# PengfeiRen96/DIR

Measured on AMD Instinct MI355X. Metric: images/sec at 256x256 bs=64, 3 stage outputs (DIR.forward eval), higher is better.
Workload: dtype f16

## Files before the change

dir_amd/_capi.py:

```python
import ctypes as C
import os

_HERE = os.path.dirname(os.path.abspath(__file__))
LIB_PATH = os.environ.get('DIR_LIB_PATH') or os.path.join(_HERE, 'lib', 'libdir_hip.so')
_lib = None


class DirHipError(RuntimeError):
    pass


class ManoTables(C.Structure):
    _fields_ = [('shapedirs_t', C.c_void_p), ('posedirs_t', C.c_void_p), ('v_template', C.c_void_p),
                ('j_template', C.c_void_p), ('j_shapedirs', C.c_void_p), ('weights', C.c_void_p), ('hands_mean', C.c_void_p),
                ('comps', C.c_void_p), ('side', C.c_int32), ('center_idx', C.c_int32), ('root_palm', C.c_int32)]


class ManoFitHand(C.Structure):
    _fields_ = [(n, C.c_void_p) for n in ('p0', 'anchor', 'p_out', 'verts_t', 'joints_t', 'joints_conf', 'uv_t', 'uv_conf', 'verts', 'joints', 'joint_uv',
                                          'mse', 'status', 'state')]


class ManoFitOpts(C.Structure):
    _fields_ = [(n, C.c_float) for n in ('w_verts', 'w_joints', 'w_uv', 'w_pca', 'w_beta', 'w_init')] + [('lr', C.c_float * 4)] + [
# ... 24 lines not shown
class ConvSrc2(C.Structure):
    _fields_ = [(n, C.c_int32) for n in ('H', 'W', 'Cin', 'in_cstride', 'in_coff', 'stride')]


class TrainWeight(C.Structure):
    _fields_ = [(n, C.c_void_p) for n in ('w', 'fwd', 'fwd_scale', 'dgrad', 'dgrad_scale')] + [(n, C.c_int32) for n in ('Cout', 'Cin', 'kh', 'kw')] + [
        ('fwd_inv_in', C.c_float), ('dgrad_inv_in', C.c_float)]


class BneckChainParams(C.Structure):
    _fields_ = [(n, C.c_void_p) for n in ('w2', 'scale2', 'shift2', 'w3', 'scale3', 'shift3', 'w1n', 'scale1n', 'shift1n', 'wd')] + [
        ('n_next', C.c_int32), ('out_decimate', C.c_int32), ('dtype', C.c_int32)]


class BneckTailParams(C.Structure):
    _fields_ = [(n, C.c_void_p) for n in ('wstream', 'scale3', 'shift3', 'scale1n', 'shift1n')] + [('planes', C.c_int32), ('n_next', C.c_int32), ('waves', C.c_int32), ('dtype', C.c_int32)]


class ResChainParams(C.Structure):
    _fields_ = [(n, C.c_void_p) for n in ('w1', 'w2', 'w3', 'pre_scale', 'pre_shift', 'scale1', 'shift1', 'scale2', 'shift2', 'shift3')] + [
        (n, C.c_int32) for n in ('Cin', 'Cmid', 'Cout', 'dtype')]


class GemmDesc(C.Structure):
    _fields_ = [(n, C.c_int32) for n in ('M', 'N', 'K', 'lda', 'ldb', 'ldc', 'trans_a', 'trans_b', 'accumulate', 'batch')] + \
               [(n, C.c_int64) for n in ('stride_a', 'stride_b', 'stride_c')]


class GemmGroups(C.Structure):
    _fields_ = [(n, C.c_int32) for n in ('ny', 'nx', 'reduce', 'reserved')] + [(n, C.c_int64) for n in ('a_y', 'a_x', 'b_y', 'b_x', 'c_y', 'c_x')]


class TokenMlp(C.Structure):
    _fields_ = [(n, C.c_void_p) for n in ('w1t', 's1', 'b1', 'w2t', 'b2')]


class PgcnLayer(C.Structure):
    _fields_ = [(n, C.c_void_p) for n in ('W', 'e1', 'bias', 'bn_scale', 'bn_shift')] + [('relu', C.c_int32), ('w_dtype', C.c_int32)]


class SteBlock(C.Structure):
    _fields_ = [(n, C.c_void_p) for n in ('ln1_w', 'ln1_b', 'qkv_wt', 'qkv_b', 'proj_wt', 'proj_b', 'ln2_w', 'ln2_b',
                                          'fc1_wt', 'fc1_b', 'fc2_wt', 'fc2_b')]


class SteParams(C.Structure):
# ... 59 lines not shown
    _fields_ = [(n, C.c_void_p) for n in ('para', 'cam_px', 'raw_verts', 'raw_joints', 'raw_joints_px', 'smoothed', 'verts', 'joints', 'joints_px',
                                          'updated', 'state')]


class ManoParaSmoothOpts(C.Structure):
    _fields_ = [(n, C.c_double) for n in ('fps', 'min_cutoff', 'beta', 'd_cutoff', 'rot_speed_scale', 'cam_speed_scale')] + [
        ('max_gap', C.c_int32), ('shape_frames', C.c_int32)]


MANO_PARA_SMOOTH_FIELDS = ('measures', 'y1', 'y2', 'x1', 'x2', 'prev', 'vel', 'n_shape', 'age', 'run', 'count')


class GuardState(C.Structure):
    _fields_ = [('sumsq', C.c_double), ('norm', C.c_double), ('bc1', C.c_double), ('applied', C.c_longlong), ('skipped', C.c_longlong),
                ('skipped_in_row', C.c_longlong), ('clipped', C.c_longlong), ('coef', C.c_float), ('bc2_sqrt', C.c_float),
                ('nonfinite', C.c_int32), ('skip', C.c_int32), ('reserved', C.c_int32 * 2)]


class RenderLights(C.Structure):
    _fields_ = [('ambient', C.c_float * 3), ('diffuse', C.c_float * 3), ('specular', C.c_float * 3), ('location', C.c_float * 3),
                ('shininess', C.c_float)]


ABI_VERSION = 54
DT_F32, DT_BF16, DT_F16X3, DT_F16X1, DT_F16X3P, DT_F16X1P, DT_F16 = 0, 1, 3, 4, 5, 6, 7
CONV_RELU, CONV_PRE_RELU = 1, 2

_p, _i = C.c_void_p, C.c_int
_SIGNATURES = {
    'dir_abi_version': (C.c_int, []),
    'dir_last_error': (C.c_char_p, []),
    'dir_device_info': (C.c_int, [C.c_char_p, _i, C.POINTER(C.c_int)]),
    'dir_launch_log_reset': (None, []),
    'dir_launch_log_get': (C.c_int, [C.c_char_p, _i]),
    'dir_launch_log_note': (None, [C.c_char_p, C.c_longlong]),
    'dir_probe_launch': (C.c_longlong, [_i, _p, C.c_longlong, _i, _p]),
    'dir_conv2d_forward': (C.c_int, [C.POINTER(ConvDesc), _p, _p, _p, _p, _p, _p, _p, _p, _p]),
    'dir_conv2d_forward_stats': (C.c_int, [C.POINTER(ConvDesc), _p, _p, _p, _p, _p, _p, _p, _p, _p, C.POINTER(C.c_int), _p]),
    'dir_conv2d_forward_masked': (C.c_int, [C.POINTER(ConvDesc), _p, _p, _p, _p, _p, _p, _p, _p, _p, _p]),
    'dir_conv2d_forward_ex': (C.c_int, [C.POINTER(ConvDesc), _p, _p, _p, _p, _p, _p, _p, _p, _p, C.POINTER(ConvBnBwd), C.POINTER(C.c_int), _p]),
    'dir_add_upsampled': (C.c_int, [_p, _p, _i, _i, _i, _i, _i, _i, _i, _p]),
    'dir_fuse_sum': (C.c_int, [_p, _p, _p, _p, _i, _i, _i, _i, _i, _i, _i, _p]),
    'dir_pack_f16x3_weights': (C.c_int, [_p, _p, _p, _p, _i, _i, _p]),
    'dir_train_pack_conv_weights': (C.c_int, [_p, _p, _i, _i, _p]),
    'dir_gemm_f32_splitk_workspace_bytes': (C.c_longlong, [C.POINTER(GemmDesc)]),
    'dir_gemm_f32_splitk': (C.c_int, [C.POINTER(GemmDesc), _p, _p, _p, _p, _p, C.c_longlong, _p]),
    'dir_axpy_multi_f32': (C.c_int, [_p, _p, _p, _i, C.c_float, _p]),
    'dir_split_f16_forward': (C.c_int, [_p, _p, C.c_longlong, _i, _i, _i, _p, _p, _i, C.c_float, _i, _p]),
    'dir_stem_prep': (C.c_int, [_p, _p, _i, _i, _i, _i, _i, _i, _i, _p]),
    'dir_stem_prep_s2d': (C.c_int, [_p, _p, _i, _i, _i, _i, _i, _i, _p]),
    'dir_image_normalize_forward': (C.c_int, [_p, _p, C.POINTER(C.c_float), C.POINTER(C.c_float), _i, _i, _i, _p]),
    'dir_stem_prep_s2d_u8': (C.c_int, [_p, _p, C.POINTER(C.c_float), C.POINTER(C.c_float), _i, _i, _i, _i, _i, _i, _p]),
    'dir_adamw_step': (C.c_int, [_p, _p, _p, _p, C.c_longlong, C.c_double, C.c_double, C.c_double, C.c_double, C.c_double,
                                 C.c_longlong, _p]),
    'dir_grad_norm_workspace_bytes': (C.c_longlong, [C.c_longlong]),
    'dir_grad_guard': (C.c_int, [_p, C.c_longlong, C.c_double, _i, C.c_double, C.c_double, _p, C.c_longlong, _p, _p]),
    'dir_adamw_guarded_step': (C.c_int, [_p, _p, _p, _p, _p, C.c_longlong, C.c_double, C.c_double, C.c_double, C.c_double, C.c_double,
                                         C.c_double, _p, _p]),
    'dir_stage_losses_backward': (C.c_int, [C.POINTER(LossPred), C.POINTER(LossTarget), C.c_float, _p, C.POINTER(C.c_void_p * 2),
                                            C.POINTER(C.c_void_p * 2), C.POINTER(LossPredGrad), _i, _p]),
    'dir_dense_losses_backward_workspace_bytes': (C.c_longlong, [_i, _i]),
    'dir_dense_losses_backward': (C.c_int, [_p, _p, _p, _p, C.POINTER(C.c_float), C.c_float, _p, _p, C.c_longlong, _p, _p, _i, _i, _i, _i, _p]),
    'dir_stage_losses_forward': (C.c_int, [C.POINTER(LossPred), C.POINTER(LossTarget), C.c_float, _p, _p, _i, _p]),
    'dir_dense_losses_workspace_bytes': (C.c_longlong, [_i, _i]),
    'dir_dense_losses_forward': (C.c_int, [_p, _p, _p, _p, C.POINTER(C.c_float), C.c_float, _p, C.c_longlong, _p, _i, _i, _i, _i, _p]),
    'dir_bottleneck_chain_forward': (C.c_int, [C.POINTER(BneckChainParams), _p, _p, _p, _p, _p, _i, _i, _i, _p]),
    'dir_bottleneck_tail_forward': (C.c_int, [C.POINTER(BneckTailParams), _p, _p, _p, _p, C.c_longlong, _p]),
    'dir_residual_chain_supported': (C.c_int, [_i] * 11),
    'dir_residual_chain_forward': (C.c_int, [C.POINTER(ResChainParams), _p, _p, _i, _i, _i, _i, _i, _i, _i, _p]),
    'dir_stem_pool_forward': (C.c_int, [_p, _i, C.POINTER(C.c_float), C.POINTER(C.c_float), _p, _p, _p, _p, _i, _i, _i, _p]),
    'dir_stem_pool_forward_dt': (C.c_int, [_p, _i, _i, C.POINTER(C.c_float), C.POINTER(C.c_float), _p, _p, _p, _p, _i, _i, _i, _p]),
    'dir_maxpool3x3s2': (C.c_int, [_p, _p, _i, _i, _i, _i, _i, _p]),
    'dir_upsample2x_bilinear': (C.c_int, [_p, _p, _i, _i, _i, _i, _i, _i, _i, _p]),
    'dir_init_head_forward': (C.c_int, [C.POINTER(InitHeadParams), _p, _p, _p, _i, _p, _p, _p, _i, _i, _i, _i, _i, _p]),
    'dir_bone_proj_forward': (C.c_int, [_p, _p, _p, _p, _p, _p, _i, _i, C.c_float, _i, _p]),
    'dir_conv2d_dual_forward': (C.c_int, [C.POINTER(ConvDesc), _p, C.POINTER(ConvSrc2), _p, _p, _p, _p, _p]),
    'dir_conv2d_dual_scaled_forward': (C.c_int, [C.POINTER(ConvDesc), _p, C.POINTER(ConvSrc2), _p, _p, _p, _p, _p, _p]),
    'dir_conv1x1_stream_forward': (C.c_int, [C.POINTER(ConvDesc), _p, C.POINTER(ConvSrc2), _p, _p, _p, _p, _p, _p, _p, _p]),
    'dir_conv2d_as_supported': (C.c_int, [C.POINTER(ConvDesc), _i, _i]),
    'dir_conv2d_as_forward': (C.c_int, [C.POINTER(ConvDesc), _p, _p, _p, _p, _p, _p, _i, _i, _p]),
    'dir_conv2d_as_chain_supported': (C.c_int, [C.POINTER(ConvDesc), _i, _i]),
    'dir_conv2d_as_chain_forward': (C.c_int, [C.POINTER(ConvDesc), _p, _p, _p, _p, _p, _p, _p, _i, _i, _p, _i, _i, _i, _p]),
    'dir_conv2d_sparse_forward': (C.c_int, [C.POINTER(ConvDesc), _p, _p, _p, _p, _p, _p, _p, _p]),
    'dir_grid_tokens_forward': (C.c_int, [_p, _i, _i, _i, _i, _i, _p, _p, _p, _p, _p, C.POINTER(TokenMlp),
                                          C.POINTER(TokenMlp), C.POINTER(TokenMlp), _p, _p, _i, _p]),
    'dir_pgcn_stack_forward': (C.c_int, [C.POINTER(PgcnLayer), _i, _p, _p, _p, C.c_longlong, _p, _i, _p]),
    'dir_pgcn_stack_forward_pair': (C.c_int, [C.POINTER(PgcnLayer), C.POINTER(PgcnLayer), _i, _p, _p, _p, _p, _i, _p]),
    'dir_ste_forward': (C.c_int, [C.POINTER(SteParams), _p, _p, _p, _i, _p]),
    'dir_regress_forward': (C.c_int, [C.POINTER(RegressParams), _p, _p, _p, _p, _p, _p, _p, _p, _i, _p]),
    'dir_bone_fusion_scratch_bytes': (C.c_size_t, [_i]),
    'dir_bone_fusion_prepare': (C.c_int, [C.POINTER(BoneFusionParams), _p, _p, _i, _p]),
    'dir_bone_fusion_forward': (C.c_int, [C.POINTER(BoneFusionParams), _p, _p, _p, _p, _i, _i, C.c_float, _i, _i, _i, _p]),
# ... 71 lines not shown
    'dir_render_adjacency': (C.c_int, [_p, _p, C.c_longlong, _p]),
    'dir_render_vertex_normals': (C.c_int, [_p, _p, _p, _i, _p, _p]),
    'dir_render_shaded_workspace_bytes': (C.c_longlong, [_i]),
    'dir_render_joints': (C.c_int, [_p, _p, _p, _i, _i, C.c_float, C.c_float, _p]),
    'dir_render_shaded': (C.c_int, [_p, _p, _p, _p, _p, _p, _p, C.POINTER(RenderLights), _p, _i, _i, _p, C.c_longlong, _p, _p, _p, _p, _p, _p]),
    'dir_mesh_penetration': (C.c_int, [_p, _p, _p, _p, _i, _i, _i, _i, _i, _p, _p, _p, _p, _p, _p]),
    'dir_mesh_intersection_volume': (C.c_int, [_p, _p, _p, _p, _i, _i, _i, _i, _i, C.c_float, _i, _p, _p, _p, _p]),
    'dir_procrustes_align': (C.c_int, [_p, _p, _i, _i, _i, _p, _p, _p, _p]),
    'dir_point_set_nn': (C.c_int, [_p, _p, _i, _i, _i, _p, _p, _p]),
    'dir_threshold_counts': (C.c_int, [_p, C.c_longlong, _p, _i, _p, _p]),
    'dir_crop_matrices_from_boxes': (C.c_int, [_p, _i, C.c_double, _i, _p, _p, _p]),
    'dir_crop_matrices_from_meshes': (C.c_int, [_p, _p, _p, _p, _p, _i, C.c_double, _i, _p, _p, _p]),
    'dir_crop_frames': (C.c_int, [_p, C.c_longlong, _p, _p, _p, _i, _i, _p, _p, _p]),
    'dir_crop_frames_area': (C.c_int, [_p, C.c_longlong, _p, _p, _p, _i, _i, _p, _p, _p, _p]),
    'dir_one_euro_state_bytes': (C.c_longlong, [_i, _i, C.POINTER(C.c_longlong)]),
    'dir_one_euro_step': (C.c_int, [_p, _p, _i, C.POINTER(OneEuroSegment), _i, C.c_double, C.c_double, C.c_double, C.c_double, _i, _p, _p, _p, _p]),
    'dir_mano_para_smooth_state_bytes': (C.c_longlong, [C.POINTER(C.c_longlong)]),
    'dir_mano_para_smooth_step': (C.c_int, [C.POINTER(ManoTables), C.POINTER(ManoParaSmoothHand), _p, C.POINTER(ManoParaSmoothOpts), _i, _i, _p]),
}


PROFILE = None
_pending = {}
_NO_PROFILE = ('dir_conv2d_as_supported', 'dir_conv2d_as_chain_supported', 'dir_residual_chain_supported', 'dir_abi_version', 'dir_last_error', 'dir_device_info', 'dir_launch_log_reset', 'dir_launch_log_get', 'dir_launch_log_note',
               'dir_bone_fusion_scratch_bytes', 'dir_dense_losses_workspace_bytes', 'dir_dense_losses_backward_workspace_bytes',
               'dir_gemm_f32_splitk_workspace_bytes', 'dir_bn_train_workspace_bytes', 'dir_bn_sync_workspace_bytes', 'dir_bn_frozen_workspace_bytes', 'dir_jpeg_planes_bytes', 'dir_render_workspace_bytes', 'dir_render_adjacency_bytes', 'dir_render_shaded_workspace_bytes', 'dir_colsum_workspace_bytes', 'dir_conv2d_wgrad_workspace_bytes', 'dir_conv2d_wgrad_f16x3_workspace_bytes',
               'dir_one_euro_state_bytes', 'dir_mano_para_smooth_state_bytes', 'dir_grad_norm_workspace_bytes')


def annotate(**kw):
    if PROFILE is not None:
        _pending.update(kw)


class _ProfLib(object):
    def __init__(self, l):
        self._l = l

    def __getattr__(self, name):
        fn = getattr(self._l, name)
        if name in _NO_PROFILE:
            return fn
        import torch

        def call(*args):
            e0, e1 = torch.cuda.Event(enable_timing=True), torch.cuda.Event(enable_timing=True)
            self._l.dir_launch_log_reset()
# ... 58 lines not shown
```

dir_amd/engine.py:

```python
import ctypes as C
import math
import json
import os
import threading

import torch

from . import _capi
from ._capi import CONV_PRE_RELU, CONV_RELU, DT_BF16, DT_F16, DT_F16X1, DT_F16X1P, DT_F16X3, DT_F16X3P, DT_F32, ConvDesc
from .packing import pack_as_weights, pack_stream_weights, pack_tail_stream

F32 = torch.float32
IMAGENET_MEAN = (C.c_float * 3)(0.485, 0.456, 0.406)
IMAGENET_STD = (C.c_float * 3)(0.229, 0.224, 0.225)
class _ThreadState(threading.local):
    variant = None
    arith = None
    capture = None
    capture_fused = None
    calibrating = False
    no_out_split = False


_TLS = _ThreadState()


def _variant_for(op, B):
    return _TLS.variant if _TLS.variant is not None else op.variant.get(B, 0)


def _packing_arith():
    return _TLS.arith

# ... 359 lines not shown
    @staticmethod
    def applies(c3, c1n, dtype):
        return (dtype in HALF and c3.kh == 1 and c3.stride == 1 and c3.scale is not None and c3.cout == 4 * c3.cin
                and c1n.kh == 1 and c1n.stride == 1 and c1n.cin == c3.cout and c1n.scale is not None and c1n.pre_scale is None
                and (c3.cin, c1n.cout) in BneckTailOp.GEOMETRIES)

    def __call__(self, y2, x):
        B, H, W, P = y2.shape
        M = B * H * W
        if _TLS.capture_fused is not None:
            _TLS.capture_fused.append((self, (y2, x), {}))
        out = torch.empty(B, H, W, self.c3.cout, device=y2.device, dtype=y2.dtype)
        y1n = torch.empty(B, H, W, self.c1n.cout, device=y2.device, dtype=y2.dtype)
        if _capi.PROFILE is not None:
            c4, n2 = self.c3.cout, self.c1n.cout
            _capi.annotate(family='conv', flops=2.0 * M * (P * c4 + c4 * n2), op=self, dtype='bf16',
                           shape='M=%d tail 1x1(%d->%d)+res+1x1(->%d)' % (M, P, c4, n2),
                           bytes=(M * (P + 2 * c4 + n2) + c4 * P + n2 * c4) * 2)
        _capi.check(_capi.lib().dir_bottleneck_tail_forward(C.byref(self.params), _capi.ptr(y2), _capi.ptr(x), _capi.ptr(out), _capi.ptr(y1n), M,
                                                            _capi.stream_ptr()), 'dir_bottleneck_tail_forward')
        return out, y1n


def stem_conv_op(w, scale, shift, dtype):
    wp = torch.zeros(64, 64, 4, 1, device=w.device, dtype=F32)
    for r in range(4):
        for dy in range(2):
            ky = 2 * r + dy - 1
            if not 0 <= ky <= 6:
                continue
            for j in range(4):
                for dx in range(2):
                    kx = 2 * j + dx - 1
                    if 0 <= kx <= 6:
                        c0 = j * 16 + (dy * 2 + dx) * 4
                        wp[:, c0:c0 + 3, r, 0] = w[:, :, ky, kx]
    op = ConvOp(wp, dtype, stride=1, pad=0, scale=scale, shift=shift, relu=True)
    op.ho = op.wo = 128
    op.in_cs_override = 16
    op.alg_k = 147
    return op


class BackboneOp(object):
    fused_stem = os.environ.get('DIR_FUSED_STEM', '1') != '0'
    bneck_chain = os.environ.get('DIR_BNECK_CHAIN', '1') != '0'
    bneck_tail = os.environ.get('DIR_BNECK_TAIL', '1') != '0'

    def __init__(self, sd, p, dtype, device):
        dt = self.dtype = dtype
        self.device = device
        w = sd[p + '.conv1.weight']
        wk = torch.zeros(64, 7, 8, 4, device=w.device, dtype=F32)
        wk[:, :, :7, :3] = w.permute(0, 2, 3, 1)
        self.stem_w = wk.to(dtype if dtype in HALF else torch.bfloat16).contiguous().to(device)
        s_, h_ = bn_fold(sd, p + '.bn1')
        self.stem_scale, self.stem_shift = s_.float().contiguous().to(device), h_.float().contiguous().to(device)
        self.stem = stem_conv_op(sd[p + '.conv1.weight'], s_, h_, dt)
        self.layers = []
        for li, n in enumerate((3, 4, 6, 3), start=1):
            blocks = []
            for b in range(n):
                q = '%s.layer%d.%d' % (p, li, b)
                stride = 2 if (b == 0 and li > 1) else 1
                s1, h1 = bn_fold(sd, q + '.bn1')
                s2, h2 = bn_fold(sd, q + '.bn2')
                s3, h3 = bn_fold(sd, q + '.bn3')
                blk = dict(c1=ConvOp(sd[q + '.conv1.weight'], dt, scale=s1, shift=h1, relu=True),
                           c2=ConvOp(sd[q + '.conv2.weight'], dt, stride=stride, pad=1, scale=s2, shift=h2, relu=True),
                           c3=ConvOp(sd[q + '.conv3.weight'], dt, scale=s3, shift=h3, relu=True))
# ... 5 lines not shown
                    blk['c2'].link_split(blk['c3'])
                blocks.append(blk)
            self.layers.append(blocks)
        if self.bneck_chain:
            l1 = self.layers[0]
            for i, blk in enumerate(l1):
                nxt = l1[i + 1]['c1'] if i + 1 < len(l1) else self.layers[1][0]['c1']
                if 'dual' in blk:
                    if BneckChainOp.applies(blk['c2'], None, nxt, dt, dual=blk['dual']):
                        blk['chain'] = BneckChainOp(blk['c2'], None, nxt, dual=blk['dual'])
                elif BneckChainOp.applies(blk['c2'], blk['c3'], nxt, dt):
                    blk['chain'] = BneckChainOp(blk['c2'], blk['c3'], nxt)

        if self.bneck_tail:
            for li in (1, 2):
                blocks = self.layers[li]
                for i, blk in enumerate(blocks):
                    if 'dual' in blk or 'chain' in blk:
                        continue
                    nxt = blocks[i + 1]['c1'] if i + 1 < len(blocks) else self.layers[li + 1][0]['c1']
                    if BneckTailOp.applies(blk['c3'], nxt, dt):
                        blk['tail'] = BneckTailOp(blk['c3'], nxt)

    def __call__(self, img):
        L, dt, dev = _capi.lib(), self.dtype, self.device
        B = img.shape[0]
        if self.fused_stem and dt in HALF:
            x = torch.empty(B, 64, 64, 64, device=dev, dtype=dt)
            u8 = img.dtype == torch.uint8
            _ann('stem', 2.0 * B * 128 * 128 * 64 * 147, img.numel() * img.element_size() + x.numel() * 2 + self.stem_w.numel() * 2,
                 'B=%d 7x7/2 conv + bn + relu + maxpool' % B)
            _capi.check(L.dir_stem_pool_forward_dt(_capi.ptr(img), 2 if u8 else 0, _dt(dt), IMAGENET_MEAN, IMAGENET_STD, _capi.ptr(self.stem_w),
                                                _capi.ptr(self.stem_scale), _capi.ptr(self.stem_shift), _capi.ptr(x), B, 256, 256,
                                                _capi.stream_ptr()), 'dir_stem_pool_forward')
            return self._layers(x)
        Hs, Ws = 131, 132
        xp = torch.empty(B, Hs, Ws, 16, device=dev, dtype=dt)
        _ann('stem', 0, img.numel() * img.element_size() + xp.numel() * xp.element_size(), 'B=%d space-to-depth staging' % B)
        if img.dtype == torch.uint8:
            _capi.check(L.dir_stem_prep_s2d_u8(_capi.ptr(img), _capi.ptr(xp), IMAGENET_MEAN, IMAGENET_STD, B, 256, 256, Hs, Ws,
                                               _dt(dt), _capi.stream_ptr()), 'dir_stem_prep_s2d_u8')
        else:
            _capi.check(L.dir_stem_prep_s2d(_capi.ptr(img), _capi.ptr(xp), B, 256, 256, Hs, Ws, _dt(dt), _capi.stream_ptr()),
                        'dir_stem_prep_s2d')
        s1 = self.stem(xp)
        x = torch.empty(B, 64, 64, 64, device=dev, dtype=dt)
        _ann('stem', 0, (s1.numel() + x.numel()) * x.element_size(), 'B=%d maxpool 3x3/2' % B)
        _capi.check(L.dir_maxpool3x3s2(_capi.ptr(s1), _capi.ptr(x), B, 128, 128, 64, _dt(dt), _capi.stream_ptr()),
                    'dir_maxpool3x3s2')
        return self._layers(x)

    decimate_c1 = os.environ.get('DIR_DECIMATE_C1', '1') != '0'

    def _layers(self, x):
        feats = []
        y1 = None
        x_dec = False
        for li, blocks in enumerate(self.layers):
            for bi, blk in enumerate(blocks):
                if 'chain' in blk:
                    dec = (self.decimate_c1 and li == 0 and bi == len(blocks) - 1 and blk['chain'].c1n is not None and 'dual' in self.layers[1][0]
                           and self.layers[1][0]['dual'].stride2 == 2 and 'chain' not in self.layers[1][0] and not _TLS.no_out_split)
                    x, y1 = blk['chain'](y1 if y1 is not None else blk['c1'](x), x, decimate=dec)
                    x_dec = dec
                    continue
                if 'tail' in blk and (x.shape[0] * x.shape[1] * x.shape[2]) % 64 == 0:
                    x, y1 = blk['tail'](blk['c2'](y1 if y1 is not None else blk['c1'](x)), x)
                elif 'dual' in blk:
                    x, y1 = blk['dual'](blk['c2'](y1 if y1 is not None else blk['c1'](x)), x, x_decimated=x_dec), None
                    x_dec = False
                else:
                    x, y1 = blk['c3'](blk['c2'](y1 if y1 is not None else blk['c1'](x)), residual=x), None
            feats.append(None if x_dec else x)
        return feats


def backbone_standalone(module, x, compute_dtype=torch.float32):
    _capi.require_cuda(x)
    if module.training:
        raise NotImplementedError('dir_amd implements the inference path (eval-mode BatchNorm); call .eval()')
    sd = {'b.' + k: v.detach() for k, v in module.state_dict().items()}
    op = BackboneOp(sd, 'b', compute_dtype, x.device)
    op.decimate_c1 = False
    with torch.cuda.device(x.device):
        feats = op(_capi.f32c(x.detach()))
    return [f.permute(0, 3, 1, 2).float() for f in feats]


# ... 810 lines not shown
```

dir_amd/packing.py:

```python
import torch


def pack_as_weights(w_ohwi, A):
    N, kh, kw, Cin = w_ohwi.shape
    assert N % (128 * A) == 0 and Cin % 64 == 0
    nt = kh * kw
    dev = w_ohwi.device
    w = w_ohwi.reshape(N, nt * Cin)
    lane = torch.arange(64, device=dev)
    l32, h = lane & 31, lane >> 5
    e = torch.arange(8, device=dev)
    g, wv, st, ks, cb = torch.meshgrid(torch.arange(N // (128 * A), device=dev), torch.arange(4, device=dev), torch.arange(nt * Cin // 64, device=dev),
                                       torch.arange(4, device=dev), torch.arange(A, device=dev), indexing='ij')
    row = (g * (128 * A) + (wv * A + cb) * 32)[..., None] + l32
    slab, tap = st // nt, st % nt
    k0 = (tap * Cin + 64 * slab + 8 * ks)[..., None] + 32 * h
    return w[row[..., None], k0[..., None] + e].contiguous()


def pack_stream_weights(w_nk, dtype=torch.bfloat16):
    N, K = w_nk.shape
    assert N % 128 == 0 and K % 64 == 0
    return pack_as_weights(w_nk.detach().to(dtype).reshape(N, 1, 1, K), 2 if N % 256 == 0 else 1)


def pack_tail_stream(w3, w1n, waves=8, dtype=torch.bfloat16):
    out_dev = w3.device
    w3 = w3.detach().float().reshape(w3.shape[0], -1).cpu()
    w1n = w1n.detach().float().reshape(w1n.shape[0], -1).cpu()
    C4, P = w3.shape
    N2 = w1n.shape[0]
    assert w1n.shape[1] == C4 and C4 == 4 * P and C4 % 512 == 0 and N2 in (128, 256)
    dev = w3.device
    lane = torch.arange(64, device=dev)
    l32, h, l16, g16 = lane & 31, lane >> 5, lane & 15, lane >> 4
    e = torch.arange(8, device=dev)
    KBS = P // 16
    out = []
    if waves == 4:
        ncc = N2 // 128
        for hf in range(C4 // 512):
            for w in range(4):
                for cb in range(4):
                    for ks in range(KBS):
                        out.append(w3[(hf * 512 + 128 * w + 32 * cb + l32)[:, None], (16 * ks + 8 * h)[:, None] + e])
                for ks in range(32):
# ... 18 lines not shown
```

include/dir_hip.h:

```cpp
#ifndef DIR_HIP_H
#define DIR_HIP_H

#include <stddef.h>
#include <stdint.h>

#ifdef __cplusplus
extern "C" {
#endif

#define DIR_OK 0
#define DIR_E_INVALID (-1)
#define DIR_E_LAUNCH (-2)
#define DIR_E_NODEVICE (-3)

#define DIR_ABI_VERSION 54

int dir_abi_version(void);
const char* dir_last_error(void);
int dir_device_info(char* arch_host, int arch_len, int* num_cu_host);
void dir_launch_log_reset(void);
int dir_launch_log_get(char* buf_host, int len);
void dir_launch_log_note(const char* name, long long times);
long long dir_probe_launch(int mode, void* buf, long long bytes, int iters, void* stream);

typedef struct dir_mano_tables {
    const float* shapedirs_t;
    const float* posedirs_t;
    const float* v_template;
    const float* j_template;
    const float* j_shapedirs;
    const float* weights;
    const float* hands_mean;
    const float* comps;
    int32_t side;
    int32_t center_idx;
    int32_t root_palm;
} dir_mano_tables;

// ... 392 lines not shown
    const float* scale1n; const float* shift1n;
    int32_t planes;
    int32_t n_next;
    int32_t waves;
    int32_t dtype;
} dir_bneck_tail_params;
int dir_bottleneck_tail_forward(const dir_bneck_tail_params* p, const void* y2, const void* residual, void* out, void* y1_next,
                                long long M, void* stream);

typedef struct dir_res_chain_params {
    const void* w1; const void* w2; const void* w3;
    const float* pre_scale; const float* pre_shift;
    const float* scale1; const float* shift1;
    const float* scale2; const float* shift2;
    const float* shift3;
    int32_t Cin, Cmid, Cout;
    int32_t dtype;
} dir_res_chain_params;
int dir_residual_chain_supported(int dtype, int Cin, int Cmid, int Cout, int B, int H, int W, int in_cstride, int in_coff, int out_cstride,
                                 int out_coff);
int dir_residual_chain_forward(const dir_res_chain_params* p, const void* x, void* out, int B, int H, int W, int in_cstride, int in_coff,
                               int out_cstride, int out_coff, void* stream);

typedef struct dir_loss_pred {
    const float* joint_uv[2];
    const float* mesh_uv[2];
    const float* proj[2];
    const float* joint_xyz[2];
    const float* mesh_xyz[2];
    const float* offset;
} dir_loss_pred;
typedef struct dir_loss_target {
    const float* joint_2d[2];
    const float* mesh_2d[2];
    const float* joint_3d[2];
    const float* mesh_3d[2];
    const float* center[2];
    const int32_t* faces[2];
    int32_t c2, n_faces;
} dir_loss_target;
int dir_stage_losses_forward(const dir_loss_pred* pred_host, const dir_loss_target* gt_host, float coord_weight, double* scratch,
                             float* out13, int B, void* stream);
long long dir_dense_losses_workspace_bytes(int B, int S);
int dir_dense_losses_forward(const float* seg_logits, const float* dense_pred, const float* gt_seg, const float* gt_dense,
                             const float* class_weight_host, float dense_weight, void* workspace, long long workspace_bytes,
                             float* out3, int B, int S, int H, int W, void* stream);
// ... 166 lines not shown
```

Before: 28200.

## Fuse layer3 bottleneck 3x3 conv, 1x1 expand, residual and next 1x1 into one kernel

Adds a persistent HIP kernel for layer3 bottleneck blocks (256 planes, 16-wide maps). It computes the 3x3 conv on a haloed row patch in LDS, then the 1x1 expand with BN, residual add and ReLU, then optionally the next block's 1x1 reduce, all in one kernel. Weights are streamed through a register ring and tiles are kept in LDS. This removes the intermediate y2 global round-trip and several launches per block. In exchange the kernel is highly specialized, with large LDS use and one block per CU, and falls back to the old path when the shape is unsupported.

```diff
diff --git a/dir_amd/_capi.py b/dir_amd/_capi.py
--- a/dir_amd/_capi.py
+++ b/dir_amd/_capi.py
@@ -70,6 +70,11 @@
         (n, C.c_int32) for n in ('Cin', 'Cmid', 'Cout', 'dtype')]
 
 
+class BneckBlockParams(C.Structure):
+    _fields_ = [(n, C.c_void_p) for n in ('wstream', 'scale2', 'shift2', 'scale3', 'shift3', 'scale1n', 'shift1n')] + [
+        (n, C.c_int32) for n in ('planes', 'n_next', 'dtype')]
+
+
 class GemmDesc(C.Structure):
     _fields_ = [(n, C.c_int32) for n in ('M', 'N', 'K', 'lda', 'ldb', 'ldc', 'trans_a', 'trans_b', 'accumulate', 'batch')] + \
                [(n, C.c_int64) for n in ('stride_a', 'stride_b', 'stride_c')]
@@ -175,7 +180,7 @@
                 ('shininess', C.c_float)]
 
 
-ABI_VERSION = 54
+ABI_VERSION = 55
 DT_F32, DT_BF16, DT_F16X3, DT_F16X1, DT_F16X3P, DT_F16X1P, DT_F16 = 0, 1, 3, 4, 5, 6, 7
 CONV_RELU, CONV_PRE_RELU = 1, 2
 
@@ -221,6 +226,8 @@
     'dir_bottleneck_tail_forward': (C.c_int, [C.POINTER(BneckTailParams), _p, _p, _p, _p, C.c_longlong, _p]),
     'dir_residual_chain_supported': (C.c_int, [_i] * 11),
     'dir_residual_chain_forward': (C.c_int, [C.POINTER(ResChainParams), _p, _p, _i, _i, _i, _i, _i, _i, _i, _p]),
+    'dir_bottleneck_block_supported': (C.c_int, [_i] * 6),
+    'dir_bottleneck_block_forward': (C.c_int, [C.POINTER(BneckBlockParams), _p, _p, _p, _p, _i, _i, _i, _p]),
     'dir_stem_pool_forward': (C.c_int, [_p, _i, C.POINTER(C.c_float), C.POINTER(C.c_float), _p, _p, _p, _p, _i, _i, _i, _p]),
     'dir_stem_pool_forward_dt': (C.c_int, [_p, _i, _i, C.POINTER(C.c_float), C.POINTER(C.c_float), _p, _p, _p, _p, _i, _i, _i, _p]),
     'dir_maxpool3x3s2': (C.c_int, [_p, _p, _i, _i, _i, _i, _i, _p]),
@@ -338,7 +345,7 @@
 
 PROFILE = None
 _pending = {}
-_NO_PROFILE = ('dir_conv2d_as_supported', 'dir_conv2d_as_chain_supported', 'dir_residual_chain_supported', 'dir_abi_version', 'dir_last_error', 'dir_device_info', 'dir_launch_log_reset', 'dir_launch_log_get', 'dir_launch_log_note',
+_NO_PROFILE = ('dir_conv2d_as_supported', 'dir_conv2d_as_chain_supported', 'dir_residual_chain_supported', 'dir_bottleneck_block_supported', 'dir_abi_version', 'dir_last_error', 'dir_device_info', 'dir_launch_log_reset', 'dir_launch_log_get', 'dir_launch_log_note',
                'dir_bone_fusion_scratch_bytes', 'dir_dense_losses_workspace_bytes', 'dir_dense_losses_backward_workspace_bytes',
                'dir_gemm_f32_splitk_workspace_bytes', 'dir_bn_train_workspace_bytes', 'dir_bn_sync_workspace_bytes', 'dir_bn_frozen_workspace_bytes', 'dir_jpeg_planes_bytes', 'dir_render_workspace_bytes', 'dir_render_adjacency_bytes', 'dir_render_shaded_workspace_bytes', 'dir_colsum_workspace_bytes', 'dir_conv2d_wgrad_workspace_bytes', 'dir_conv2d_wgrad_f16x3_workspace_bytes',
                'dir_one_euro_state_bytes', 'dir_mano_para_smooth_state_bytes', 'dir_grad_norm_workspace_bytes')
diff --git a/dir_amd/csrc/l3_chain.hip b/dir_amd/csrc/l3_chain.hip
--- /dev/null
+++ b/dir_amd/csrc/l3_chain.hip
@@ -0,0 +1,323 @@
+#include "conv_common.h"
+
+namespace dir {
+namespace {
+
+using convk::bf16_t;
+using convk::f16s_t;
+using convk::f32x16;
+using convk::Half;
+
+constexpr int P = 256, C4 = 1024;
+constexpr int TM = 64;
+constexpr int HC = 512;
+constexpr int NTHR = 512;
+constexpr int TPITCH = HC * 2 + 16;
+constexpr int YPITCH = P * 2 + 16;
+constexpr int PROW = 9728;
+constexpr int PATCH = 6 * PROW;
+constexpr int R0 = TM * TPITCH > PATCH ? TM * TPITCH : PATCH;
+constexpr int GRP = 8;
+constexpr int NAF = 144;
+constexpr int NBF = 32;
+
+struct L3Args {
+    const bf16_t* y1; const bf16_t* res; bf16_t* out; bf16_t* y1n;
+    const uint4* wstream;
+    const float* sc2; const float* sh2; const float* sc3; const float* sh3; const float* sc1n; const float* sh1n;
+    int H, tiles_per_img, ntiles;
+};
+
+template <typename H> __device__ __forceinline__ void unpack4(uint2 v, float (&f)[4]) {
+    convk::unpack2<H>(v.x, f[0], f[1]);
+    convk::unpack2<H>(v.y, f[2], f[3]);
+}
+
+template <int V> struct IC : std::integral_constant<int, V> {};
+
+template <int N2, typename H>
+__global__ __launch_bounds__(NTHR, 1) void l3_chain_kernel(L3Args a) {
+    convk::half_kernel_init<H>();
+    constexpr bool NEXT = N2 != 0;
+    constexpr int NCF = NEXT ? HC / 16 : 0;
+    constexpr int NUF = NBF + NCF;
+    constexpr int NF = NAF + 2 * NUF;
+    constexpr int NGA = NAF / GRP, NGU = NUF / GRP;
+    static_assert(NAF % (2 * GRP) == 0 && NUF % (2 * GRP) == 0 && (N2 == 0 || N2 == 256), "l3_chain_kernel: the ring slot of a group must be compile-time");
+    __shared__ __attribute__((aligned(16))) char s_r0[R0];
+    __shared__ __attribute__((aligned(16))) char s_y2[TM * YPITCH];
+    __shared__ __attribute__((aligned(16))) float s_ss[2 * P + 2 * C4 + 2 * N2 + 4];
+    char* const s_t = s_r0;
+    const int tid = threadIdx.x, lane = tid & 63, wave = __builtin_amdgcn_readfirstlane(tid >> 6);
+    const int l32 = lane & 31, h = lane >> 5;
+
+    const int nblk = gridDim.x;
+    int t0, tstep, tend;
+    if ((nblk & 7) == 0 && a.ntiles % 8 == 0) {
+        const int per = a.ntiles >> 3;
+        t0 = (blockIdx.x & 7) * per + (blockIdx.x >> 3); tstep = nblk >> 3; tend = ((blockIdx.x & 7) + 1) * per;
+    } else { t0 = blockIdx.x; tstep = nblk; tend = a.ntiles; }
+    if (t0 >= tend) return;
+
+    const __amdgpu_buffer_rsrc_t wrs = __builtin_amdgcn_make_buffer_rsrc((void*)a.wstream, 0, 8 * NF * 1024, 0x00020000);
+    const int wv = (wave * NF * 64 + lane) * 16;
+    convk::u32x4 ring[2][GRP];
+    auto ring_load = [&](auto Slot, auto F0) {
+        constexpr int slot = decltype(Slot)::value, f0 = decltype(F0)::value;
+#pragma unroll
+        for (int i = 0; i < GRP; ++i) ring[slot][i] = __builtin_bit_cast(convk::u32x4, __builtin_amdgcn_raw_buffer_load_b128(wrs, wv, (f0 + i) * 1024, 0));
+    };
+    ring_load(IC<0>{}, IC<0>{});
+
+    for (int i = tid; i < P; i += NTHR) { s_ss[i] = a.sc2[i]; s_ss[P + i] = a.sh2[i]; }
+    for (int i = tid; i < C4; i += NTHR) { s_ss[2 * P + i] = a.sc3[i]; s_ss[2 * P + C4 + i] = a.sh3[i]; }
+    if constexpr (NEXT) {
+        for (int i = tid; i < N2; i += NTHR) { s_ss[2 * P + 2 * C4 + i] = a.sc1n[i]; s_ss[2 * P + 2 * C4 + N2 + i] = a.sh1n[i]; }
+    }
+    const float* const s_sc3 = s_ss + 2 * P;
+    const float* const s_sh3 = s_ss + 2 * P + C4;
+
+    uint4 xr[2][2][2];
+    auto res_fetch = [&](int tile, int half) {
+#pragma unroll
+        for (int pb = 0; pb < 2; ++pb) {
+            const bf16_t* rp = a.res + ((long long)tile * TM + 32 * pb + l32) * C4 + half * HC + 64 * wave + 8 * h;
+#pragma unroll
+            for (int cb = 0; cb < 2; ++cb)
+#pragma unroll
+                for (int j = 0; j < 2; ++j) xr[cb][pb][j] = *reinterpret_cast<const uint4*>(rp + 32 * cb + 16 * j);
+        }
+    };
+
+    f32x16 accc[2];
+    uint4 bop[2][2];
+    auto act_read = [&](auto F, auto Set) {
+        constexpr int f = decltype(F)::value, set = decltype(Set)::value;
+        if constexpr (f < NBF) {
+            constexpr int ks = f % 16;
+            constexpr int koff = NEXT ? 32 * ks : 128 * (ks >> 2) + 16 * (ks & 3);
+#pragma unroll
+            for (int pb = 0; pb < 2; ++pb)
+                bop[set][pb] = *reinterpret_cast<const uint4*>(s_y2 + (32 * pb + l32) * YPITCH + koff + (NEXT ? 16 : 64) * h);
+        } else {
+            constexpr int fc = f - NBF;
+#pragma unroll
+            for (int pb = 0; pb < 2; ++pb) bop[set][pb] = *reinterpret_cast<const uint4*>(s_t + (32 * pb + l32) * TPITCH + 32 * fc + 16 * h);
+        }
+    };
+
+    for (int t = t0; t < tend; t += tstep) {
+        const int img = t / a.tiles_per_img, trow = (t - img * a.tiles_per_img) * 4;
+
+        {
+            const int px = tid >> 5, ch = tid & 31;
+            uint4 pv[6];
+#pragma unroll
+            for (int i = 0; i < 6; ++i) {
+                const int iy = trow - 1 + i, iyc = min(max(iy, 0), a.H - 1);
+                pv[i] = *reinterpret_cast<const uint4*>(a.y1 + (((long long)img * a.H + iyc) * 16 + px) * P + ch * 8);
+                if (iy != iyc) pv[i] = make_uint4(0u, 0u, 0u, 0u);
+            }
+            res_fetch(t, 0);
+#pragma unroll
+            for (int i = 0; i < 6; ++i) *reinterpret_cast<uint4*>(s_r0 + i * PROW + (px + 1) * YPITCH + ch * 16) = pv[i];
+            if (tid < 384) *reinterpret_cast<uint4*>(s_r0 + (tid >> 6) * PROW + ((tid >> 5) & 1) * 17 * YPITCH + ch * 16) = make_uint4(0u, 0u, 0u, 0u);
+        }
+        __syncthreads();
+
+        {
+            f32x16 acc[2];
+#pragma unroll
+            for (int j = 0; j < 2; ++j)
+#pragma unroll
+                for (int r = 0; r < 16; ++r) acc[j][r] = 0.f;
+            const char* bB = s_r0 + (l32 >> 4) * PROW + (l32 & 15) * YPITCH + 64 * h;
+            auto bread = [&](auto I) {
+                constexpr int i = decltype(I)::value, s = i >> 2, ks = i & 3, slab = s / 9, tap = s % 9, ky = tap / 3, kx = tap % 3;
+#pragma unroll
+                for (int j = 0; j < 2; ++j) bop[i & 1][j] = *reinterpret_cast<const uint4*>(bB + (ky + 2 * j) * PROW + kx * YPITCH + slab * 128 + 16 * ks);
+            };
+            bread(IC<0>{});
+            [&]<int... G>(std::integer_sequence<int, G...>) {
+                (([&] {
+                     constexpr int grp = G, slot = G & 1;
+                     __builtin_amdgcn_sched_barrier(0);
+                     ring_load(IC<slot ^ 1>{}, IC<(G + 1) * GRP>{});
+                     [&]<int... I>(std::integer_sequence<int, I...>) {
+                         (([&] {
+                              constexpr int i = grp * GRP + I;
+                              if constexpr (i + 1 < NAF) bread(IC<i + 1>{});
+                              __builtin_amdgcn_sched_barrier(0);
+#pragma unroll
+                              for (int j = 0; j < 2; ++j) acc[j] = Half<H>::mfma32(ring[slot][I], bop[i & 1][j], acc[j]);
+                          }()),
+                          ...);
+                     }(std::make_integer_sequence<int, GRP>{});
+                 }()),
+                 ...);
+            }(std::make_integer_sequence<int, NGA>{});
+#pragma unroll
+            for (int j = 0; j < 2; ++j)
+#pragma unroll
+                for (int q = 0; q < 4; ++q) {
+                    const int c0 = 32 * wave + 8 * q + 4 * h;
+                    const float4 sc = *reinterpret_cast<const float4*>(s_ss + c0);
+                    const float4 sh = *reinterpret_cast<const float4*>(s_ss + P + c0);
+                    uint2 o;
+                    o.x = Half<H>::pack2_relu(fmaf(acc[j][4 * q], sc.x, sh.x), fmaf(acc[j][4 * q + 1], sc.y, sh.y));
+                    o.y = Half<H>::pack2_relu(fmaf(acc[j][4 * q + 2], sc.z, sh.z), fmaf(acc[j][4 * q + 3], sc.w, sh.w));
+                    *reinterpret_cast<uint2*>(s_y2 + (32 * j + l32) * YPITCH + c0 * 2) = o;
+                }
+        }
+        __syncthreads();
+
+        auto unit = [&](auto HF) {
+            constexpr int hf = decltype(HF)::value;
+            constexpr bool last_half = hf == 1;
+            constexpr int fbase = NAF + hf * NUF;
+            f32x16 accb[2];
+            if constexpr (NEXT && hf == 0) {
+#pragma unroll
+                for (int pb = 0; pb < 2; ++pb)
+#pragma unroll
+                    for (int r = 0; r < 16; ++r) accc[pb][r] = 0.f;
+            }
+            act_read(IC<0>{}, IC<0>{});
+            [&]<int... G>(std::integer_sequence<int, G...>) {
+                (([&] {
+                     constexpr int grp = G, slot = G & 1;
+                     constexpr int fnext = G + 1 < NGU ? fbase + (G + 1) * GRP : last_half ? 0 : fbase + NUF;
+                     ring_load(IC<slot ^ 1>{}, IC<fnext>{});
+                     [&]<int... I>(std::integer_sequence<int, I...>) {
+                         (([&] {
+                              constexpr int f = grp * GRP + I, set = f & 1;
+                              if constexpr (f + 1 < NUF && f + 1 != NBF) act_read(IC<f + 1>{}, IC<set ^ 1>{});
+                              if constexpr (f < NBF) {
+                                  constexpr int cb = f / 16, ks = f - cb * 16;
+                                  if constexpr (ks == 0) {
+#pragma unroll
+                                      for (int pb = 0; pb < 2; ++pb)
+#pragma unroll
+                                          for (int r = 0; r < 16; ++r) accb[pb][r] = 0.f;
+                                  }
+#pragma unroll
+                                  for (int pb = 0; pb < 2; ++pb) accb[pb] = Half<H>::mfma32(ring[slot][I], bop[set][pb], accb[pb]);
+                                  if constexpr (ks == 15) {
+#pragma unroll
+                                      for (int q = 0; q < 4; ++q) {
+                                          const int cl = 64 * wave + 32 * cb + 8 * q + 4 * h;
+                                          const float4 sc = *reinterpret_cast<const float4*>(s_sc3 + hf * HC + cl);
+                                          const float4 sh = *reinterpret_cast<const float4*>(s_sh3 + hf * HC + cl);
+#pragma unroll
+                                          for (int pb = 0; pb < 2; ++pb) {
+                                              float v[4] = {fmaf(accb[pb][4 * q], sc.x, sh.x), fmaf(accb[pb][4 * q + 1], sc.y, sh.y),
+                                                            fmaf(accb[pb][4 * q + 2], sc.z, sh.z), fmaf(accb[pb][4 * q + 3], sc.w, sh.w)};
+                                              float rv[4];
+                                              {
+                                                  const uint4 c = xr[cb][pb][q >> 1];
+                                                  const auto sx = __builtin_amdgcn_permlane32_swap(c.x, c.z, false, false);
+                                                  const auto sy = __builtin_amdgcn_permlane32_swap(c.y, c.w, false, false);
+                                                  unpack4<H>(make_uint2(sx[q & 1], sy[q & 1]), rv);
+                                              }
+#pragma unroll
+                                              for (int e = 0; e < 4; ++e) v[e] += rv[e];
+                                              uint2 o;
+                                              o.x = Half<H>::pack2_relu(v[0], v[1]);
+                                              o.y = Half<H>::pack2_relu(v[2], v[3]);
+                                              *reinterpret_cast<uint2*>(s_t + (32 * pb + l32) * TPITCH + cl * 2) = o;
+                                          }
+                                          __builtin_amdgcn_sched_barrier(0);
+                                      }
+                                  }
+                                  if constexpr (f == NBF - 1) {
+                                      __syncthreads();
+                                      if constexpr (NEXT) act_read(IC<NBF>{}, IC<set ^ 1>{});
+                                      if constexpr (!last_half) res_fetch(t, hf + 1);
+#pragma unroll
+                                      for (int i = 0; i < TM * (HC / 8) / NTHR; ++i) {
+                                          const int c = tid + NTHR * i;
+                                          *reinterpret_cast<uint4*>(a.out + ((long long)t * TM + (c >> 6)) * C4 + hf * HC + (c & 63) * 8) =
+                                              *reinterpret_cast<const uint4*>(s_t + (c >> 6) * TPITCH + (c & 63) * 16);
+                                          if (i & 1) __builtin_amdgcn_sched_barrier(0);
+                                      }
+                                  }
+                              } else {
+#pragma unroll
+                                  for (int pb = 0; pb < 2; ++pb) accc[pb] = Half<H>::mfma32(ring[slot][I], bop[set][pb], accc[pb]);
+                              }
+                              __builtin_amdgcn_sched_barrier(0);
+                          }()),
+                          ...);
+                     }(std::make_integer_sequence<int, GRP>{});
+                 }()),
+                 ...);
+            }(std::make_integer_sequence<int, NGU>{});
+            if constexpr (NEXT && last_half) {
+                const float* const s_sc1 = s_ss + 2 * P + 2 * C4;
+#pragma unroll
+                for (int pb = 0; pb < 2; ++pb) {
+                    uint2 o[4];
+#pragma unroll
+                    for (int q = 0; q < 4; ++q) {
+                        const int c0 = 32 * wave + 8 * q + 4 * h;
+                        const float4 sc = *reinterpret_cast<const float4*>(s_sc1 + c0);
+                        const float4 sh = *reinterpret_cast<const float4*>(s_sc1 + N2 + c0);
+                        o[q].x = Half<H>::pack2_relu(fmaf(accc[pb][4 * q], sc.x, sh.x), fmaf(accc[pb][4 * q + 1], sc.y, sh.y));
+                        o[q].y = Half<H>::pack2_relu(fmaf(accc[pb][4 * q + 2], sc.z, sh.z), fmaf(accc[pb][4 * q + 3], sc.w, sh.w));
+                    }
+#pragma unroll
+                    for (int j = 0; j < 2; ++j) {
+                        const auto dx = __builtin_amdgcn_permlane32_swap(o[2 * j].x, o[2 * j + 1].x, false, false);
+                        const auto dy = __builtin_amdgcn_permlane32_swap(o[2 * j].y, o[2 * j + 1].y, false, false);
+                        *reinterpret_cast<uint4*>(a.y1n + ((long long)t * TM + 32 * pb + l32) * N2 + 32 * wave + 16 * j + 8 * h) = make_uint4(dx[0], dy[0], dx[1], dy[1]);
+                    }
+                }
+            }
+            __syncthreads();
+        };
+        unit(IC<0>{});
+        unit(IC<1>{});
+    }
+}
+
+}
+}
+
+extern "C" int dir_bottleneck_block_supported(int dtype, int planes, int n_next, int B, int H, int W) {
+    if (dtype != DIR_DT_BF16 && dtype != DIR_DT_F16) return 0;
+    if (planes != dir::P || !(n_next == 256 || n_next == 0)) return 0;
+    if (B <= 0 || H <= 0 || W != 16 || H % 4) return 0;
+    if ((long long)B * (H / 4) >= (1ll << 31)) return 0;
+    return 1;
+}
+
+extern "C" int dir_bottleneck_block_forward(const dir_bneck_block_params* p, const void* y1, const void* residual, void* out, void* y1_next,
+                                            int B, int H, int W, void* stream) {
+    using namespace dir;
+    DIR_REQUIRE(p && y1 && residual && out, "dir_bottleneck_block_forward: null pointer");
+    DIR_REQUIRE(p->wstream && p->scale2 && p->shift2 && p->scale3 && p->shift3, "dir_bottleneck_block_forward: missing parameters");
+    DIR_REQUIRE(dir_bottleneck_block_supported(p->dtype, p->planes, p->n_next, B, H, W),
+                "dir_bottleneck_block_forward: unsupported (bf16 / f16 storage, planes 256, n_next 256 or 0, W = 16, H a multiple of 4)");
+    DIR_REQUIRE(p->n_next == 0 || (y1_next && p->scale1n && p->shift1n), "dir_bottleneck_block_forward: null pointer (the fused next conv1 needs y1_next, scale1n and shift1n)");
+    L3Args a;
+    a.y1 = (const convk::bf16_t*)y1; a.res = (const convk::bf16_t*)residual; a.out = (convk::bf16_t*)out; a.y1n = (convk::bf16_t*)y1_next;
+    a.wstream = (const uint4*)p->wstream;
+    a.sc2 = p->scale2; a.sh2 = p->shift2; a.sc3 = p->scale3; a.sh3 = p->shift3; a.sc1n = p->scale1n; a.sh1n = p->shift1n;
+    a.H = H; a.tiles_per_img = H / 4; a.ntiles = B * (H / 4);
+    static int num_cu = 0;
+    if (!num_cu) {
+        int dev = 0; hipDeviceProp_t pr;
+        num_cu = (hipGetDevice(&dev) == hipSuccess && hipGetDeviceProperties(&pr, dev) == hipSuccess) ? pr.multiProcessorCount : 256;
+    }
+    const int grid = a.ntiles < num_cu ? a.ntiles : num_cu;
+    hipStream_t s = (hipStream_t)stream;
+    const bool f16 = p->dtype == DIR_DT_F16;
+    if (p->n_next == 256) {
+        if (f16) DIR_LAUNCH((l3_chain_kernel<256, f16s_t>), dim3(grid), dim3(NTHR), 0, s, a);
+        else DIR_LAUNCH((l3_chain_kernel<256, bf16_t>), dim3(grid), dim3(NTHR), 0, s, a);
+    } else {
+        if (f16) DIR_LAUNCH((l3_chain_kernel<0, f16s_t>), dim3(grid), dim3(NTHR), 0, s, a);
+        else DIR_LAUNCH((l3_chain_kernel<0, bf16_t>), dim3(grid), dim3(NTHR), 0, s, a);
+    }
+    return check_launch("dir_bottleneck_block_forward");
+}
diff --git a/dir_amd/engine.py b/dir_amd/engine.py
--- a/dir_amd/engine.py
+++ b/dir_amd/engine.py
@@ -8,7 +8,7 @@
 
 from . import _capi
 from ._capi import CONV_PRE_RELU, CONV_RELU, DT_BF16, DT_F16, DT_F16X1, DT_F16X1P, DT_F16X3, DT_F16X3P, DT_F32, ConvDesc
-from .packing import pack_as_weights, pack_stream_weights, pack_tail_stream
+from .packing import pack_as_weights, pack_l3_stream, pack_stream_weights, pack_tail_stream
 
 F32 = torch.float32
 IMAGENET_MEAN = (C.c_float * 3)(0.485, 0.456, 0.406)
@@ -414,6 +414,49 @@
         return out, y1n
 
 
+class BneckBlockOp(object):
+
+    def __init__(self, c2, c3, c1n=None, covered=None):
+        self.c2, self.c3, self.c1n = c2, c3, c1n
+        self.covers = (covered if covered is not None else c3,)
+        self.cout, self.cin, self.kh, self.kw, self.stride = c3.cout, c2.cin, 3, 3, 1
+        self.variant = c2.variant
+        self.stream = pack_l3_stream(c2.w, c3.w.reshape(c3.cout, c3.cin), None if c1n is None else c1n.w.reshape(c1n.cout, c1n.cin), dtype=c2.dtype)
+        n = (lambda t: None) if c1n is None else _capi.ptr
+        self.params = _capi.BneckBlockParams(_capi.ptr(self.stream), _capi.ptr(c2.scale), _capi.ptr(c2.shift), _capi.ptr(c3.scale), _capi.ptr(c3.shift),
+                                             n(c1n.scale if c1n is not None else None), n(c1n.shift if c1n is not None else None),
+                                             c2.cout, c1n.cout if c1n is not None else 0, _dt(c2.dtype))
+
+    @staticmethod
+    def applies(c2, c3, c1n, dtype):
+        ok = (dtype in HALF and c2.arith is None and (c2.kh, c2.kw, c2.stride, c2.pad, c2.cin, c2.cout) == (3, 3, 1, 1, 256, 256)
+              and c2.scale is not None and c2.pre_scale is None and (c2.flags & CONV_RELU)
+              and (c3.kh, c3.stride, c3.cin, c3.cout) == (1, 1, 256, 1024) and c3.scale is not None and c3.pre_scale is None and (c3.flags & CONV_RELU))
+        return bool(ok and (c1n is None or ((c1n.kh, c1n.stride, c1n.cin, c1n.cout) == (1, 1, 1024, 256) and c1n.scale is not None
+                                            and c1n.pre_scale is None and (c1n.flags & CONV_RELU))))
+
+    def supported(self, y1, x):
+        B, H, W, Pn = y1.shape
+        return bool(y1.dtype == self.c2.dtype and x.dtype == y1.dtype and y1.is_contiguous() and x.is_contiguous() and Pn == 256
+                    and tuple(x.shape) == (B, H, W, 1024)
+                    and _capi.lib().dir_bottleneck_block_supported(_dt(y1.dtype), 256, self.params.n_next, B, H, W))
+
+    def __call__(self, y1, x):
+        B, H, W, _ = y1.shape
+        if _TLS.capture_fused is not None:
+            _TLS.capture_fused.append((self, (y1, x), {}))
+        out = torch.empty(B, H, W, 1024, device=y1.device, dtype=y1.dtype)
+        y1n = torch.empty(B, H, W, 256, device=y1.device, dtype=y1.dtype) if self.c1n is not None else None
+        if _capi.PROFILE is not None:
+            m, n2 = B * H * W, self.params.n_next
+            _capi.annotate(family='conv', flops=2.0 * m * (256 * 9 * 256 + 256 * 1024 + 1024 * n2), op=self.c2, covers=self.covers, dtype='bf16',
+                           shape='M=%d block 3x3(256)+1x1(->1024)+res%s' % (m, '+1x1(->%d)' % n2 if n2 else ''),
+                           bytes=(m * (256 + 2 * 1024 + n2) + 256 * 9 * 256 + 1024 * 256 + n2 * 1024) * 2)
+        _capi.check(_capi.lib().dir_bottleneck_block_forward(C.byref(self.params), _capi.ptr(y1), _capi.ptr(x), _capi.ptr(out), _capi.ptr(y1n), B, H, W,
+                                                             _capi.stream_ptr()), 'dir_bottleneck_block_forward')
+        return out, y1n
+
+
 def stem_conv_op(w, scale, shift, dtype):
     wp = torch.zeros(64, 64, 4, 1, device=w.device, dtype=F32)
     for r in range(4):
@@ -438,6 +481,7 @@
     fused_stem = os.environ.get('DIR_FUSED_STEM', '1') != '0'
     bneck_chain = os.environ.get('DIR_BNECK_CHAIN', '1') != '0'
     bneck_tail = os.environ.get('DIR_BNECK_TAIL', '1') != '0'
+    l3_chain = os.environ.get('DIR_L3_CHAIN', '1') != '0'
 
     def __init__(self, sd, p, dtype, device):
         dt = self.dtype = dtype
@@ -489,6 +533,14 @@
                     if BneckTailOp.applies(blk['c3'], nxt, dt):
                         blk['tail'] = BneckTailOp(blk['c3'], nxt)
 
+        if self.l3_chain:
+            for i, blk in enumerate(self.layers[2]):
+                if 'dual' in blk or 'chain' in blk:
+                    continue
+                nxt = blk['tail'].c1n if 'tail' in blk else None
+                if BneckBlockOp.applies(blk['c2'], blk['c3'], nxt, dt):
+                    blk['block'] = BneckBlockOp(blk['c2'], blk['c3'], nxt, covered=blk.get('tail'))
+
     def __call__(self, img):
         L, dt, dev = _capi.lib(), self.dtype, self.device
         B = img.shape[0]
@@ -531,6 +583,11 @@
                     x, y1 = blk['chain'](y1 if y1 is not None else blk['c1'](x), x, decimate=dec)
                     x_dec = dec
                     continue
+                if 'block' in blk and self.l3_chain:
+                    y1 = y1 if y1 is not None else blk['c1'](x)
+                    if blk['block'].supported(y1, x):
+                        x, y1 = blk['block'](y1, x)
+                        continue
                 if 'tail' in blk and (x.shape[0] * x.shape[1] * x.shape[2]) % 64 == 0:
                     x, y1 = blk['tail'](blk['c2'](y1 if y1 is not None else blk['c1'](x)), x)
                 elif 'dual' in blk:
diff --git a/dir_amd/packing.py b/dir_amd/packing.py
--- a/dir_amd/packing.py
+++ b/dir_amd/packing.py
@@ -22,6 +22,18 @@
     N, K = w_nk.shape
     assert N % 128 == 0 and K % 64 == 0
     return pack_as_weights(w_nk.detach().to(dtype).reshape(N, 1, 1, K), 2 if N % 256 == 0 else 1)
+
+
+def pack_l3_stream(w2_ohwi, w3, w1n=None, dtype=torch.bfloat16):
+    w2 = w2_ohwi.detach().to(dtype)
+    w3 = w3.detach().reshape(w3.shape[0], -1).to(dtype)
+    assert tuple(w2.shape) == (256, 3, 3, 256) and tuple(w3.shape) == (1024, 256)
+    a = pack_as_weights(w2, 1).reshape(8, 144, 64, 8)
+    if w1n is not None:
+        u = pack_tail_stream(w3, w1n, 8, dtype=dtype).to(w2.device).reshape(2, 8, 64, 64, 8)
+    else:
+        u = pack_as_weights(w3.reshape(1024, 1, 1, 256), 1).reshape(2, 8, 32, 64, 8)
+    return torch.cat([a, u[0], u[1]], 1).contiguous()
 
 
 def pack_tail_stream(w3, w1n, waves=8, dtype=torch.bfloat16):
diff --git a/include/dir_hip.h b/include/dir_hip.h
--- a/include/dir_hip.h
+++ b/include/dir_hip.h
@@ -13,7 +13,7 @@
 #define DIR_E_LAUNCH (-2)
 #define DIR_E_NODEVICE (-3)
 
-#define DIR_ABI_VERSION 54
+#define DIR_ABI_VERSION 55
 
 int dir_abi_version(void);
 const char* dir_last_error(void);
@@ -452,6 +452,19 @@
 int dir_residual_chain_forward(const dir_res_chain_params* p, const void* x, void* out, int B, int H, int W, int in_cstride, int in_coff,
                                int out_cstride, int out_coff, void* stream);
 
+typedef struct dir_bneck_block_params {
+    const void* wstream;
+    const float* scale2; const float* shift2;
+    const float* scale3; const float* shift3;
+    const float* scale1n; const float* shift1n;
+    int32_t planes;
+    int32_t n_next;
+    int32_t dtype;
+} dir_bneck_block_params;
+int dir_bottleneck_block_supported(int dtype, int planes, int n_next, int B, int H, int W);
+int dir_bottleneck_block_forward(const dir_bneck_block_params* p, const void* y1, const void* residual, void* out, void* y1_next,
+                                 int B, int H, int W, void* stream);
+
 typedef struct dir_loss_pred {
     const float* joint_uv[2];
     const float* mesh_uv[2];
```

Result: faster. 28630 (median of 6 runs) (+1.5%).
